# rrruko/squigly-trace

Hardware: AMD Instinct MI355X
Metric: Msamples/s (whole node) at 1080p/256spp on data/scene.obj (higher is better)
Workload: dtype f32; 1 GPU; data/scene.obj 1920x1080 @ 256 spp (BASELINE configs[1]), rows sharded over 1 GPU(s) in blocks of 2, RGB8 all_gather_into_tensor; row_block=2, nonblack_pixels=629970

## Files before the change

### squigly-trace_amd/csrc/sq_device.hip

```cpp
#include <hip/hip_runtime.h>

#include <algorithm>
#include <atomic>
#include <cmath>
#include <cstdlib>
#include <cstring>
#include <mutex>
#include <string>
#include <chrono>
#include <thread>
#include <vector>

#include "../../include/squigly_hip.h"
#include "../../include/squigly_host.h"
#include "sq_error.h"
#include "sq_pack.h"
#include "sq_kernels_lane.h"
#include "sq_kernels_wave.h"
#include "sq_kernels_trace.h"

#define SQ_HIP(expr)                                                                             \
    do {                                                                                         \
        hipError_t e_ = (expr);                                                                  \
        if (e_ != hipSuccess) return sq_set_error("%s failed: %s", #expr, hipGetErrorString(e_)); \
    } while (0)

constexpr int kOneshotRowBlock = 2;

struct RngTable { uint32_t* words = nullptr; size_t bytes = 0; int64_t cover = 0; hipEvent_t filled = nullptr; };
struct sq_device_scene {
    int device = 0;
    SceneView view{};
    void* d_arena = nullptr;
    int height = 0; bool small_index = false; int n_cu = 256;
    Level1Cull level1{};
    int shortcut_depth = 0;
    Work work{}; void* d_work = nullptr; size_t work_bytes = 0; int64_t work_pixels = 0, work_slots = 0;
    std::vector<std::pair<hipEvent_t, hipEvent_t>> pending;
    double total_ms = 0; int64_t launches = 0;
    Options opt;
    const char* last_kernel = "sq_trace_rays";
    sq_plan plan{}; bool has_plan = false;
    hipStream_t aux = nullptr; std::vector<hipEvent_t> events;
    float* d_cams = nullptr; int64_t cams_cap = 0;
    float* d_px_sum2 = nullptr; int64_t px_sum2_cap = 0;
    RngTable rng{};
    std::vector<sq_light> lights{ sq_light{ { 0.0f, 3.0f, -1.0f }, { 2.0f, 2.0f, 2.0f } } };
    bool lights_set = false, lights_staged = false;
    float* d_lights = nullptr; float* cast_carry = nullptr;
    int32_t depth = 3;
    void* d_deep = nullptr; size_t deep_bytes = 0;
    sq_sky sky{}; bool sky_set = false;
};

extern "C" int sq_scene_upload(const sq_scene* sc, int32_t device, sq_device_scene** out) {
    if (sq_check_scene_args(sc, out)) return 1;
    int ndev = 0;
    if (hipGetDeviceCount(&ndev) != hipSuccess || ndev < 1) return sq_set_error("no HIP device available (this library has no CPU fallback)");
    if (device < 0 || device >= ndev) return sq_set_error("device %d outside 0..%d", device, ndev - 1);
    PackedScene P;
    if (sq_pack_scene(*sc, P)) return 1;
    SQ_HIP(hipSetDevice(device));
    sq_device_scene* s = new sq_device_scene;
    s->device = device; s->height = P.height; s->small_index = P.small_index; s->shortcut_depth = P.shortcut_depth; s->level1 = P.level1;
    hipDeviceProp_t prop;
    if (hipGetDeviceProperties(&prop, device) == hipSuccess && prop.multiProcessorCount > 0) s->n_cu = prop.multiProcessorCount;
    SceneView& v = s->view;
    auto arrays = [&](auto&& f) {
        f(v.branches, P.branches, false); f(v.leaves, P.leaves, false); f(v.tris, P.tris, false); f(v.tri_mat, P.tri_mat, false);
        f(v.surfs, P.surfs, false); f(v.mats, P.mats, false); f(v.verts4, P.verts4, false); f(v.trix, P.trix, false);
        f(v.rbranch, P.rbranch, false); f(v.emitters, P.emitters, false);
        f(v.cull_child, P.cull_child, true); f(v.cull_child16, P.cull_child16, true); f(v.branches_m, P.branches_m, true);
    };
    auto slot = [](size_t bytes) { return ((bytes ? bytes : 16) + 255) & ~(size_t)255; };
    size_t arena_bytes = 0;
    arrays([&](auto&, const auto& vec, bool optional) { if (!optional || !vec.empty()) arena_bytes += slot(vec.size() * sizeof(vec[0])); });
    if (hipMalloc(&s->d_arena, arena_bytes) != hipSuccess) { sq_scene_free(s); return sq_set_error("hipMalloc(%zu) for the scene failed", arena_bytes); }
    std::vector<unsigned char> staging(arena_bytes, 0);
    size_t off = 0;
    arrays([&](auto& member, const auto& vec, bool optional) {
        if (optional && vec.empty()) return;
        const size_t bytes = vec.size() * sizeof(vec[0]);
        if (bytes) std::memcpy(staging.data() + off, vec.data(), bytes);
        member = reinterpret_cast<std::remove_reference_t<decltype(member)>>((const char*)s->d_arena + off);
        off += slot(bytes);
    });
    if (hipMemcpy(s->d_arena, staging.data(), arena_bytes, hipMemcpyHostToDevice) != hipSuccess) { sq_scene_free(s); return sq_set_error("hipMemcpy H2D of the scene failed"); }
    if (P.trix.empty()) v.trix = nullptr;
    for (int c = 0; c < 3; ++c) { v.root_lo[c] = sc->root.lo[c]; v.root_hi[c] = sc->root.hi[c]; }
    v.root_ref = P.root_ref; v.packed_leaves = P.packed_leaves; v.rroot = P.rroot;
    v.n_branches = P.nb; v.n_leaves = P.nl; v.n_tris = sc->n_tris; v.n_mats = sc->n_mats; v.n_verts = P.n_verts; v.n_emitters = P.n_emitters;
    v.height = P.height; v.nonneg_materials = P.nonneg_materials; v.finite_geometry = P.finite_geometry;
    v.cull_o2max = P.cull_limits[0]; v.cull_d2min = P.cull_limits[1]; v.cull_d2max = P.cull_limits[2];
    v.rtail = nullptr; v.incremental_ok = 0;
    *out = s;
    return 0;
}

namespace {
struct CachedBlock { void* ptr = nullptr; size_t bytes = 0; };
std::mutex g_cache_mutex;
CachedBlock g_cache[64];
void* cache_take(int device, size_t bytes, size_t* got) {
    std::lock_guard<std::mutex> lock(g_cache_mutex);
    CachedBlock& c = g_cache[device & 63];
    if (!c.ptr || c.bytes < bytes) return nullptr;
    void* p = c.ptr; *got = c.bytes; c = CachedBlock{};
    return p;
}
void cache_give(int device, void* ptr, size_t bytes) {
    void* drop = ptr;
    {
        std::lock_guard<std::mutex> lock(g_cache_mutex);
        CachedBlock& c = g_cache[device & 63];
        if (bytes > c.bytes) { drop = c.ptr; c.ptr = ptr; c.bytes = bytes; }
    }
    if (drop) (void)hipFree(drop);
}
RngTable g_rng_cache[64];
void rng_free(RngTable& t) {
    if (t.words) (void)hipFree(t.words);
    if (t.filled) (void)hipEventDestroy(t.filled);
    t = RngTable{};
}
bool rng_cache_take(int device, int64_t cover, RngTable* out) {
    std::lock_guard<std::mutex> lock(g_cache_mutex);
    RngTable& c = g_rng_cache[device & 63];
    if (!c.words || c.cover < cover) return false;
    *out = c; c = RngTable{};
    return true;
}
void rng_cache_give(int device, RngTable& t) {
    RngTable drop = t;
    t = RngTable{};
    {
        std::lock_guard<std::mutex> lock(g_cache_mutex);
        RngTable& c = g_rng_cache[device & 63];
        if (drop.cover > c.cover) std::swap(drop, c);
    }
    rng_free(drop);
}
}
extern "C" void sq_release_cached_memory(void) {
    for (int d = 0; d < 64; ++d) {
        size_t got = 0;
        void* p = cache_take(d, 0, &got);
        RngTable t;
// ... 1029 lines not shown
```

### squigly-trace_amd/csrc/sq_frame.h

```cpp
#pragma once
#include "sq_plan.h"
#include "sq_scene.h"

using sq::f3;
using namespace sqd;

struct Frame {
    float cam_pos[3]; float cam_rot[9];
    int32_t samples, w, h, cast;
    int32_t row_block, shard, n_shards, local_rows;
    int32_t tile_rows, tiles_x;
    float* out_avg; uint8_t* out_rgb;
    int32_t k_begin, k_end;
    float* sum;
    int32_t diag;
    int32_t n_views, view_pixels;
    const float* cams;
    const uint8_t* mask; float* sum2; int32_t* count;
};
struct RayFrame : Frame {
    const float* ray_org; const float* ray_dir; const long long* ray_seed;
};
template <int SRC> using FrameOf = std::conditional_t<SRC == kSrcRays, RayFrame, Frame>;
constexpr int kCamWords = 12;
// ... 85 lines not shown
template <typename T> __device__ __forceinline__ T sky_arg() { return T{}; }
template <typename T> __device__ __forceinline__ const T& sky_arg(const T& k) { return k; }
__device__ __forceinline__ float sky_t(f3 d) {
    const float n = sq::fsqrt((d.x * d.x + d.y * d.y) + d.z * d.z);
    const float u = d.z / n;
    return 0.5f * u + 0.5f;
}
__device__ __forceinline__ f3 sky_at(const Sky& K, float t) {
    return sq::mk(K.down[0] + t * (K.up[0] - K.down[0]), K.down[1] + t * (K.up[1] - K.down[1]), K.down[2] + t * (K.up[2] - K.down[2]));
}
__device__ __forceinline__ void store_fold(const Frame& F, long long pix, f3 sum) {
    if (F.sum) { float* o = F.sum + pix * 3; o[0] = sum.x; o[1] = sum.y; o[2] = sum.z; }
    const f3 avg = sq::scale(1 / (float)F.k_end, sum);
    if (F.out_avg) { float* o = F.out_avg + pix * 3; o[0] = avg.x; o[1] = avg.y; o[2] = avg.z; }
    if (F.out_rgb) tonemap(avg, F.out_rgb + pix * 3);
}
template <bool AD>
__device__ __forceinline__ void store_miss_sky(const Frame& F, long long pix, const Sky& K, f3 d0) {
    const f3 c = sky_at(K, sky_t(d0));
    f3 sum = fold_start(F, pix);
    for (int k = F.k_begin; k < F.k_end; ++k) sum = sum + c;
    if constexpr (AD) {
        if (F.sum2) {
            f3 sum2 = fold_start2(F, pix);
            for (int k = F.k_begin; k < F.k_end; ++k) sum2 = sum2 + c * c;
            float* o = F.sum2 + pix * 3; o[0] = sum2.x; o[1] = sum2.y; o[2] = sum2.z;
        }
        store_count(F, pix);
    }
    store_fold(F, pix, sum);
}

struct Work {
    int32_t* n_active;
    int32_t* px_pixel;
    float*   px_t0;
    int32_t* px_tri0;
    float*   px_sum;
    float*   px_mt;
    int32_t* px_mtri;
    uint8_t* state;
    float4*  org;
    float4*  dir;
    int32_t* tri1;
    int32_t* head[2];
    unsigned long long* stats;
    int64_t  slot_capacity;
    float*   px_sum2;
};
constexpr uint8_t kDone = 0, kRay1 = 1, kMirror = 2, kRay2 = 3;

constexpr int kDiagGauge = 24, kDiagWaves = 25, kDiagStartBeside = 26, kDiagEndBeside = 27;
constexpr int kStatLevel1Culled = 28;

__device__ __forceinline__ int wave_append(int32_t* counter, bool want) {
    const unsigned long long m = sq_ballot(want);
    if (m == 0) return -1;
    const int lane = threadIdx.x & 63;
    const int leader = __ffsll((long long)m) - 1;
    int base = 0;
    if (lane == leader) base = atomicAdd(counter, __popcll(m));
    base = __shfl(base, leader);
    return want ? base + __popcll(m & ((1ull << lane) - 1ull)) : -1;
}

template <bool AD>
__device__ __forceinline__ void store_active(const Frame& F, const Work& W, int a, long long pix, float t, int tri) {
    W.px_pixel[a] = (int32_t)pix; W.px_t0[a] = t; W.px_tri0[a] = tri;
    const f3 s0 = fold_start(F, pix);
    W.px_sum[3 * a] = s0.x; W.px_sum[3 * a + 1] = s0.y; W.px_sum[3 * a + 2] = s0.z;
    if constexpr (AD) {
        if (F.sum2) { const f3 q0 = fold_start2(F, pix); W.px_sum2[3 * a] = q0.x; W.px_sum2[3 * a + 1] = q0.y; W.px_sum2[3 * a + 2] = q0.z; }
        store_count(F, pix);
    }
}
template <bool AD>
__device__ __forceinline__ void store_miss(const Frame& F, long long pix) {
    if constexpr (AD) store_live_miss(F, pix); else store_miss_sum(F, pix);
}

constexpr int kRngRun = 4;
constexpr size_t kRngPad = 256;
struct RngView { const uint32_t* words; long long cover; };

__device__ __forceinline__ f3 level0_radiance(const Surface& s0) { return s0.surf * sq::mk(0, 0, 0) + s0.emit; }
struct Shade1 { f3 surf, emit; };
__device__ __forceinline__ Shade1 shade1_of(const SceneView& S, int tri) {
    const float4* q = S.surfs + 3 * (size_t)tri;
    return Shade1{ sq::mk(q[1].x, q[1].y, q[1].z), sq::mk(q[2].x, q[2].y, q[2].z) };
}
__device__ __forceinline__ f3 level1_radiance(const Surface& s0, const Shade1& s1) {
    const f3 L1 = s1.surf * sq::mk(0, 0, 0) + s1.emit;
    return s0.surf * L1 + s0.emit;
}

constexpr int kMaxDepth = kDeepestPath;
__device__ __forceinline__ uint32_t tf_word(const uint64_t c[4], int i) {
    const uint64_t w = i < 2 ? c[0] : i < 4 ? c[1] : i < 6 ? c[2] : c[3];
    return (i & 1) ? (uint32_t)(w >> 32) : (uint32_t)w;
}
__device__ __forceinline__ f3 path_radiance(const SceneView& S, const Surface& s0, const int (&tr)[kMaxDepth], f3 inner) {
    f3 L = inner;
#pragma unroll
    for (int b = kMaxDepth - 1; b >= 1; --b)
        if (tr[b] >= 0) { const Shade1 q = shade1_of(S, tr[b]); L = q.surf * L + q.emit; }
    return s0.surf * L + s0.emit;
// ... 40 lines not shown
```

### squigly-trace_amd/csrc/sq_host.cpp

```cpp
#include "../../include/squigly_host.h"
#include "sq_error.h"
#include "sq_host_types.h"
#include "sq_math.h"
#include "sq_pack.h"
#include "sq_plan.h"

#include <algorithm>
#include <cmath>
#include <cstdio>
#include <cstdlib>
#include <cstring>
#include <string>
#include <unordered_map>
#include <vector>

using sq::f3;

namespace {

struct Scanner {
    const char* s; size_t n; size_t i = 0;
    Scanner(const char* p, size_t len) : s(p), n(len) {}
    int peek() const { return i < n ? (unsigned char)s[i] : -1; }
    static bool ws(int c) { return c == ' ' || c == '\t' || c == '\n' || c == '\r' || c == '\f' || c == '\v'; }
// ... 713 lines not shown
                vmax2 = std::max(vmax2, q);
            }
        const double vmax = std::sqrt(vmax2), omax = 2.0 * vmax * (1.0 + 1e-12);
        double g1 = 0.0;
        for (int32_t i = 0; i < sc.n_tris; ++i) {
            if (emits[(size_t)i]) continue;
            const TriNorms q = tri_norms(sc.tris[i]);
            if (!(q.P <= kLemmaPmax)) return;
            const double rho = lemma_rho(q, omax), r = 7.0 * u * q.P / eps;
            g1 = std::max(g1, rho + 1.01 * (r * (omax + vmax + rho) + rho));
        }
        const double delta1 = 4.0 * u * (2.0 * (vmax + g1) + omax) * (1.0 + 1e-6), R1 = vmax + g1 + delta1;
        if (!(R1 <= 1048576.0)) return;
        double six = 0.0;
        for (int c = 0; c < 3; ++c) { L.em_lo[c] = P.emitters.empty() ? 0.0 : 1e300; L.em_hi[c] = P.emitters.empty() ? 0.0 : -1e300; }
        for (int32_t e : P.emitters) {
            const sq_tri& t = sc.tris[e];
            const TriNorms q = tri_norms(t);
            if (!(q.P <= kLemmaPmax)) return;
            L.em_rho = std::max(L.em_rho, 32.0 * (u / eps) * q.P * (R1 + q.V0 + q.E1 + q.E2));
            six = std::max(six, 6.0 * u * (q.E1 + q.E2));
            for (const float* v : { t.v0, t.v1, t.v2 })
                for (int c = 0; c < 3; ++c) {
                    L.em_lo[c] = std::min(L.em_lo[c], (double)v[c]);
                    L.em_hi[c] = std::max(L.em_hi[c], (double)v[c]);
                }
        }
        L.em_add = six + delta1 + 1e-20;
        std::vector<float> vals;
        for (int32_t i = 0; i < sc.n_tris; ++i) vals.push_back(P.surfs[(size_t)i].reflective);
        std::sort(vals.begin(), vals.end()); vals.erase(std::unique(vals.begin(), vals.end()), vals.end());
        const size_t nv = vals.size(), nc = std::min<size_t>(nv, (size_t)kLevel1Classes);
        L.n_classes = (int32_t)nc;
        for (size_t c = 0; c < nc; ++c) {
            L.class_val[c] = vals[nv - nc + c];
            const float from = (c == 0) ? vals[0] : L.class_val[c];
            float* b = L.class_box[c];
            b[0] = b[1] = b[2] = INFINITY; b[3] = b[4] = b[5] = -INFINITY;
            for (int32_t i = 0; i < sc.n_tris; ++i) {
                if (!(P.surfs[(size_t)i].reflective >= from)) continue;
                const sq_tri& t = sc.tris[i];
                const TriNorms q = tri_norms(t);
                if (!(q.P <= kLemmaPmax)) { b[0] = b[1] = b[2] = -INFINITY; b[3] = b[4] = b[5] = INFINITY; break; }
                double m = lemma_rho(q, omax);
                m += 8.0 * u * (vmax_inf + m + omax) + 1e-20;
                for (int k = 0; k < 3; ++k) {
                    const double lo = std::min({ (double)t.v0[k], (double)t.v1[k], (double)t.v2[k] }), hi = std::max({ (double)t.v0[k], (double)t.v1[k], (double)t.v2[k] });
                    b[k] = std::min(b[k], f_down(lo - m)); b[3 + k] = std::max(b[3 + k], f_up(hi + m));
                }
            }
        }
        L.o2max = P.cull_limits[0]; L.d2min = P.cull_limits[1]; L.d2max = P.cull_limits[2];
        L.on = 1;
    }
    void geometry_flags() {
        bool fin = finite3(sc.root.lo) && finite3(sc.root.hi);
        for (const DevBranch& d : P.branches) fin = fin && finite3(d.lo) && finite3(d.hi) && finite(d.lmax) && finite(d.rmin);
        for (int32_t i = 0; i < sc.n_tris && fin; ++i) fin = finite3(sc.tris[i].v0) && finite3(sc.tris[i].v1) && finite3(sc.tris[i].v2);
        P.finite_geometry = fin;
        P.small_index = P.nb < 0x8000 && sc.n_tris < 0x8000;
        P.n_verts = (int32_t)(P.verts4.size() / 4);
    }
};

}

int sq_pack_scene(const sq_scene& sc, PackedScene& out) {
    out = PackedScene{};
    Packer k{ sc, out };
    if (validate_tree(sc, out.height, k.depth)) return 1;
    if (sc.height && sc.height != out.height) return sq_set_error("scene.height = %d but the tree has height %d", sc.height, out.height);
    k.renumber(); k.branch_boxes(); k.material_flags(); k.triangles_and_surfaces(); k.vertex_index_form(); k.resident_encoding();
    if (k.culling_tables() || k.leaf_references()) return 1;
    k.merged_records(); k.emitter_list(); k.geometry_flags(); k.level1_tables();
    return 0;
}

struct sq_packed : PackedScene {};
extern "C" int sq_scene_pack(const sq_scene* sc, sq_packed** out) {
    if (sq_check_scene_args(sc, out)) return 1;
    sq_packed* p = new sq_packed;
    if (sq_pack_scene(*sc, *p)) { delete p; return 1; }
    *out = p;
    return 0;
}
extern "C" void sq_packed_free(sq_packed* p) { delete p; }
extern "C" int sq_packed_array(const sq_packed* P, const char* name, const void** data, size_t* bytes) {
    if (!P || !name || !data || !bytes) return sq_set_error("null argument");
    bool found = false;
    auto is = [&](const char* n, const auto& v) { if (!found && !std::strcmp(name, n)) { found = true; *data = v.data(); *bytes = v.size() * sizeof(v[0]); } };
    is("branches", P->branches); is("leaves", P->leaves); is("tris", P->tris); is("tri_mat", P->tri_mat); is("surfs", P->surfs);
    is("mats", P->mats); is("verts4", P->verts4); is("trix", P->trix); is("rbranch", P->rbranch); is("emitters", P->emitters);
    is("cull_child", P->cull_child); is("cull_child16", P->cull_child16); is("branches_m", P->branches_m);
    if (!found && !std::strcmp(name, "level1")) { found = true; *data = &P->level1; *bytes = sizeof P->level1; }
    return found ? 0 : sq_set_error("no packed array '%s'", name);
}
extern "C" int sq_packed_scalar(const sq_packed* P, const char* name, int64_t* value) {
    if (!P || !name || !value) return sq_set_error("null argument");
    uint32_t lim[3]; std::memcpy(lim, P->cull_limits, sizeof lim);
    const struct { const char* name; int64_t value; } all[] = {
        { "n_branches", P->nb }, { "n_leaves", P->nl }, { "height", P->height }, { "root_ref", P->root_ref }, { "rroot", P->rroot },
        { "packed_leaves", P->packed_leaves }, { "nonneg_materials", P->nonneg_materials }, { "finite_geometry", P->finite_geometry },
        { "n_emitters", P->n_emitters }, { "n_verts", P->n_verts }, { "cull_o2max", lim[0] }, { "cull_d2min", lim[1] }, { "cull_d2max", lim[2] },
        { "small_index", P->small_index }, { "shortcut_depth", P->shortcut_depth }, { "level1_zero", P->level1_zero }, { "level1_on", P->level1.on } };
    for (const auto& s : all) if (!std::strcmp(name, s.name)) { *value = s.value; return 0; }
    return sq_set_error("no packed scalar '%s'", name);
}

extern "C" int64_t sq_rng_table_cover(int32_t w, int32_t h, int32_t samples, int64_t budget_bytes) {
    if (w < 1 || h < 1 || samples < 1 || budget_bytes < 12) return 0;
    const unsigned __int128 span = (unsigned __int128)samples * ((unsigned __int128)(w - 1) * (unsigned __int128)w + (unsigned __int128)h);
    const unsigned __int128 cap = (unsigned __int128)(budget_bytes / 12);
    return (int64_t)(span < cap ? span : cap);
}

namespace sqd {
namespace {
enum OptionKind { kAny, kRange, kBool, kSign, kIgnored };
struct OptionRow { const char* name; int64_t Options::* member; OptionKind kind; int64_t lo, hi; const char* refusal; };
const OptionRow kOptionTable[] = {
    { "timing", &Options::timing, kAny, 0, 0, nullptr },
    { "variant", &Options::variant, kRange, 1, 2, "variant must be 1 (per-pixel kernel) or 2 (wavefront)" },
    { "slots", &Options::slots, kRange, 1, 512ll << 20, "slots must be in 1..2^29" },
    { "straggler_lanes", &Options::straggler_lanes, kRange, 0, 63, "straggler_lanes must be in 0..63" },
    { "resident", &Options::resident, kBool, 0, 1, nullptr },
    { "profile", &Options::profile, kBool, 0, 1, nullptr },
    { "lds_node_kb", &Options::lds_node_kb, kRange, 0, 128, "lds_node_kb must be in 0..128" },
    { "trace_blocks_per_cu", &Options::trace_blocks_per_cu, kRange, 0, 8, "trace_blocks_per_cu must be in 0..8" },
    { "overlap", &Options::overlap, kRange, 0, 2, "overlap must be 0, 1 or 2" },
    { "rng_table_mb", &Options::rng_table_mb, kRange, 0, 1ll << 20, "rng_table_mb must be in 0..2^20" },
    { "cast_wavefront", &Options::cast_wavefront, kBool, 0, 1, nullptr },
    { "deep", &Options::deep, kBool, 0, 1, nullptr },
    { "pool", &Options::pool, kBool, 0, 1, nullptr },
    { "guided", &Options::guided, kRange, 0, 3, "guided must be in 0..3" },
    { "primary_resident", &Options::primary_resident, kBool, 0, 1, nullptr },
    { "cull", &Options::cull, kBool, 0, 1, nullptr },
    { "level1_cull", &Options::level1_cull, kBool, 0, 1, nullptr },
    { "incremental", nullptr, kIgnored, 0, 0, nullptr },
    { "primary_tiles", &Options::primary_tiles, kBool, 0, 1, nullptr },
    { "primary_pooled", &Options::primary_pooled, kBool, 0, 1, nullptr },
    { "coresidency", &Options::coresidency, kBool, 0, 1, nullptr },
    { "aux_polite", &Options::aux_polite, kRange, 0, 8, "aux_polite must be in 0..8" },
    { "trace_prio", &Options::trace_prio, kRange, 0, 3, "trace_prio must be in 0..3" },
    { "aux_low_priority", &Options::aux_low_priority, kBool, 0, 1, nullptr },
    { "descend_extra", &Options::descend_extra, kRange, 0, 16, "descend_extra must be in 0..16" },
    { "descend_lanes", &Options::descend_lanes, kRange, 1, 64, "descend_lanes must be in 1..64" },
// ... 306 lines not shown
```

### squigly-trace_amd/csrc/sq_kernels_wave.h

```cpp
#pragma once
#include "sq_frame.h"

__device__ __forceinline__ void diag_aux_wave(const Work& W, int diag, bool at_start) {
    if (!diag || (threadIdx.x & 63) != 0) return;
    const unsigned long long live = atomicAdd(&W.stats[kDiagGauge], 0ull);
    if (at_start) atomicAdd(&W.stats[kDiagWaves], 1ull);
    if (live >= (unsigned long long)diag) atomicAdd(&W.stats[at_start ? kDiagStartBeside : kDiagEndBeside], 1ull);
}

template <typename StackT, int SRC, bool AD, bool SKY, typename FrameT>
__device__ __forceinline__ void primary_body(const SceneView& S, const FrameT& F, const Work& W, const Sky& K) {
    constexpr bool MV = SRC == kSrcViews;
    extern __shared__ float4 lds_raw[];
    SQ_LDS StackT* stk = to_lds<StackT>(lds_raw) + threadIdx.x;
    const long long q = (long long)blockIdx.x * kBlock + threadIdx.x;
    int view = 0;
    long long pix;
    if constexpr (SRC == kSrcRays) pix = q < (long long)F.h ? q : -1;
    else if constexpr (MV) pix = q < primary_padded(F) * F.n_views ? primary_tile_views(F, q, view) : -1;
    else pix = q < primary_padded(F) ? primary_tile(F, q) : -1;
    bool in = pix >= 0;
    if constexpr (AD) in = in && pixel_live(F, pix);
    Hit h0; h0.tri = -1; h0.t = 0;
    f3 d0 = sq::mk(0, 0, 0);
// ... 50 lines not shown
__device__ __forceinline__ long long seed_base(const FrameT& F, const Work& W, int a, const Pixel0& P) {
    if constexpr (SRC == kSrcRays) return F.ray_seed[W.px_pixel[a]];
    else return (long long)F.samples * ((long long)P.x + (long long)P.y * (long long)F.w);
}
__device__ __forceinline__ bool absorbs(const SceneView& S, const Surface& s) {
    return S.nonneg_materials && s.surf.x == 0.0f && s.surf.y == 0.0f && s.surf.z == 0.0f;
}
__device__ __forceinline__ void finish_level1(const Work& W, long long sid, int tri1) {
    W.tri1[sid] = tri1;
    W.state[sid] = kDone;
}
__device__ __forceinline__ int2 slot_hit(const float4& org) { return make_int2(__float_as_int(org.x), __float_as_int(org.y)); }

struct RngRun { uint32_t w[3 * kRngRun]; };
__device__ __forceinline__ RngRun rng_load_run(const uint32_t* words, long long seed) {
    RngRun r;
    const uint32_t* p = words + 3 * seed;
    if ((seed & 3) == 0) {
        const uint4* q = reinterpret_cast<const uint4*>(p);
        const uint4 a = q[0], b = q[1], c = q[2];
        r.w[0] = a.x; r.w[1] = a.y; r.w[2] = a.z; r.w[3] = a.w; r.w[4] = b.x; r.w[5] = b.y; r.w[6] = b.z; r.w[7] = b.w;
        r.w[8] = c.x; r.w[9] = c.y; r.w[10] = c.z; r.w[11] = c.w;
    } else {
#pragma unroll
        for (int i = 0; i < 3 * kRngRun; ++i) r.w[i] = p[i];
    }
    return r;
}
__global__ void __launch_bounds__(kBlock) sq_rng_fill(uint32_t* words, long long quad_begin, long long quad_end) {
    for (long long q = quad_begin + (long long)blockIdx.x * kBlock + threadIdx.x; q < quad_end; q += (long long)gridDim.x * kBlock) {
        uint32_t w[3 * kRngRun];
#pragma unroll
        for (int j = 0; j < kRngRun; ++j) sq::tfgen3(q * kRngRun + j, w[3 * j], w[3 * j + 1], w[3 * j + 2]);
        uint4* o = reinterpret_cast<uint4*>(words + 3 * kRngRun * q);
        o[0] = make_uint4(w[0], w[1], w[2], w[3]); o[1] = make_uint4(w[4], w[5], w[6], w[7]); o[2] = make_uint4(w[8], w[9], w[10], w[11]);
    }
}

__device__ __forceinline__ bool halfplane_misses_box(f3 p0, f3 d1, f3 nd, const double* lo, const double* hi, double m) {
    const double px[3] = { p0.x, p0.y, p0.z }, dx[3] = { d1.x, d1.y, d1.z }, nx[3] = { nd.x, nd.y, nd.z };
    double g[3], h[3], scale = 0.0;
#pragma unroll
    for (int k = 0; k < 3; ++k) { g[k] = 0.5 * (lo[k] + hi[k]) - px[k]; h[k] = 0.5 * (hi[k] - lo[k]) + m; scale += __builtin_fabs(g[k]) + h[k]; }
    const double tol = 1e-9 * scale;
    const double N[3] = { dx[1] * nx[2] - dx[2] * nx[1], dx[2] * nx[0] - dx[0] * nx[2], dx[0] * nx[1] - dx[1] * nx[0] };
    const double dist = __builtin_fabs(N[0] * g[0] + N[1] * g[1] + N[2] * g[2]);
    const double rad = __builtin_fabs(N[0]) * h[0] + __builtin_fabs(N[1]) * h[1] + __builtin_fabs(N[2]) * h[2];
    if (dist > rad + tol) return true;
    const double f = (dx[0] * nx[0] + dx[1] * nx[1] + dx[2] * nx[2]) / (nx[0] * nx[0] + nx[1] * nx[1] + nx[2] * nx[2]);
    const double w[3] = { dx[0] - f * nx[0], dx[1] - f * nx[1], dx[2] - f * nx[2] };
    const double side = w[0] * g[0] + w[1] * g[1] + w[2] * g[2] + __builtin_fabs(w[0]) * h[0] + __builtin_fabs(w[1]) * h[1] + __builtin_fabs(w[2]) * h[2];
    return side < -tol;
}
__device__ __forceinline__ bool level1_culled(const SceneView& S, const Level1Cull& C, bool p0_ok, f3 p0, f3 d1, uint32_t n1, uint32_t n2) {
    const float eps = 0.0001f, inf = __builtin_inff();
    const f3 df = sq::mk(1.0f / d1.x, 1.0f / d1.y, 1.0f / d1.z);
    const f3 nodf = sq::mk(-p0.x * df.x, -p0.y * df.y, -p0.z * df.z);
    const float dd = sq::dot(d1, d1);
    if (!(p0_ok && finite3(d1) && finite3(df) && finite3(nodf) && dd >= C.d2min && dd <= C.d2max)) return false;
    const float un1 = sq::unit_float(n1);
    bool has = false; float b[6] = { 0, 0, 0, 0, 0, 0 };
#pragma unroll
    for (int c = kLevel1Classes - 1; c >= 0; --c) {
        if (c < C.n_classes && C.class_val[c] >= un1) {
            has = true;
#pragma unroll
            for (int k = 0; k < 6; ++k) b[k] = C.class_box[c][k];
        }
    }
    if (has && cull_slab(b, df, nodf)) return false;
    const f3 nd = random_vector(n1, n2);
    const float nn = sq::dot(nd, nd);
    if (!(nn >= C.d2min && nn <= C.d2max)) return false;
    float amin = inf;
    for (int j = 0; j < S.n_emitters; ++j) {
        const float* tp = S.tris + 9 * (size_t)S.emitters[j];
        const f3 v0 = sq::mk(tp[0], tp[1], tp[2]), e1 = sq::mk(tp[3], tp[4], tp[5]), e2 = sq::mk(tp[6], tp[7], tp[8]);
        float t_unused;
        if (moller_trumbore(p0, d1, v0, e1, e2, t_unused)) return false;
        const float a = sq::dot(e1, sq::cross(nd, e2));
        if (!(a > -eps && a < eps)) amin = sq::hmin(amin, __builtin_fabsf(a));
    }
    if (amin == inf) return true;
    if (!(amin < inf)) return false;
    return halfplane_misses_box(p0, d1, nd, C.em_lo, C.em_hi, C.em_rho * ((double)eps / (double)amin) + C.em_add);
}

template <int SRC, typename FrameT>
__device__ __forceinline__ void gen_bounce1_body(const SceneView& S, const FrameT& F, const Work& W, int k_base, int k_count, const RngView R, const Level1Cull& C) {
    const int A = *W.n_active;
    unsigned int n_culled = 0;
    diag_aux_wave(W, F.diag, true);
    const int n_runs = (k_count + kRngRun - 1) / kRngRun, runs_per_y = (n_runs + (int)gridDim.y - 1) / (int)gridDim.y;
    const int g_begin = min(n_runs, (int)blockIdx.y * runs_per_y), g_end = min(n_runs, g_begin + runs_per_y);
    for (int a = blockIdx.x * kBlock + threadIdx.x; a < A; a += gridDim.x * kBlock) {
        const Pixel0 P = load_pixel0<SRC>(S, F, W, a);
        const long long rix = seed_base<SRC>(F, W, a, P);
        if (absorbs(S, P.s0)) {
            for (int kl = g_begin * kRngRun; kl < min(k_count, g_end * kRngRun); ++kl) W.state[(long long)kl * A + a] = kDone;
            continue;
        }
        const long long first = rix + k_base;
        const bool use = R.words != nullptr && rix >= 0 && rix <= R.cover - (long long)F.samples;
        const bool p0_ok = C.on && finite3(P.p0) && sq::dot(P.p0, P.p0) <= C.o2max;
        RngRun next{};
        if (use && g_begin < g_end) next = rng_load_run(R.words, first + (long long)g_begin * kRngRun);
        for (int g = g_begin; g < g_end; ++g) {
            RngRun cur = next;
            if (use && g + 1 < g_end) next = rng_load_run(R.words, first + (long long)(g + 1) * kRngRun);
#pragma unroll 1
            for (int kl = g * kRngRun; kl < min(k_count, (g + 1) * kRngRun); ++kl) {
                const long long sid = (long long)kl * A + a;
                uint32_t n0, n1, n2;
                if (use) {
                    n0 = cur.w[0]; n1 = cur.w[1]; n2 = cur.w[2];
#pragma unroll
                    for (int i = 0; i + 3 < 3 * kRngRun; ++i) cur.w[i] = cur.w[i + 3];
                } else {
                    long long seed = first + kl;
                    asm volatile("" : "+v"(seed));
                    sq::tfgen3(seed, n0, n1, n2);
                }
                if (!scatters(P.s0, n0)) {
                    W.state[sid] = kMirror;
                    *reinterpret_cast<float2*>(reinterpret_cast<float*>(W.org + sid) + 2) = make_float2(__uint_as_float(n2), __uint_as_float(n1));
                    continue;
                }
                const f3 d1 = scatter_dir(P.d0, P.s0, n0, n1);
                if (C.on && level1_culled(S, C, p0_ok, P.p0, d1, n1, n2)) { finish_level1(W, sid, -1); ++n_culled; continue; }
                W.state[sid] = kRay1;
                W.org[sid] = make_float4(P.p0.x, P.p0.y, P.p0.z, __uint_as_float(n1));
                W.dir[sid] = make_float4(d1.x, d1.y, d1.z, __uint_as_float(n2));
            }
        }
    }
    if (C.on) {
#pragma unroll
        for (int o = 32; o > 0; o >>= 1) n_culled += __shfl_xor(n_culled, o);
        if ((threadIdx.x & 63) == 0 && n_culled) atomicAdd(&W.stats[kStatLevel1Culled], (unsigned long long)n_culled);
    }
    diag_aux_wave(W, F.diag, false);
}
constexpr int kGen1Waves = 4;
template <int SRC>
__global__ void __launch_bounds__(kBlock, kGen1Waves) sq_gen_bounce1(const SceneView S, const FrameOf<SRC> F, const Work W, int k_base, int k_count, const RngView R, const Level1Cull C) { gen_bounce1_body<SRC>(S, F, W, k_base, k_count, R, C); }

template <int SRC, typename FrameT>
__device__ __forceinline__ void mirror1_gen_body(const SceneView& S, const FrameT& F, const Work& W, long long base) {
    const int A = *W.n_active;
    for (int a = blockIdx.x * kBlock + threadIdx.x; a < A; a += gridDim.x * kBlock) {
        const Pixel0 P = load_pixel0<SRC>(S, F, W, a);
        const long long sl = base + a;
        if (absorbs(S, P.s0)) { W.state[sl] = kDone; continue; }
        const f3 d1 = mirror_dir(P.d0, P.s0);
        W.state[sl] = kRay1;
        W.org[sl] = make_float4(P.p0.x, P.p0.y, P.p0.z, 0.0f);
        W.dir[sl] = make_float4(d1.x, d1.y, d1.z, 0.0f);
    }
}
template <int SRC>
__global__ void __launch_bounds__(kBlock) sq_mirror1_gen(const SceneView S, const FrameOf<SRC> F, const Work W, long long base) { mirror1_gen_body<SRC>(S, F, W, base); }
__global__ void __launch_bounds__(kBlock) sq_mirror1_store(const Work W, long long base) {
    const int A = *W.n_active;
    for (int a = blockIdx.x * kBlock + threadIdx.x; a < A; a += gridDim.x * kBlock) {
        const bool live = W.state[base + a] == kRay1;
        const int2 hit = slot_hit(W.org[base + a]);
        W.px_mt[a] = live ? __int_as_float(hit.x) : 0.0f;
        W.px_mtri[a] = live ? hit.y : -1;
    }
}

template <int SRC, bool AD>
__global__ void __launch_bounds__(kBlock) sq_primary_gen(const FrameOf<SRC> F, const Work W, long long total) {
    if (blockIdx.x == 0 && threadIdx.x == 0) W.n_active[48] = (int32_t)total;
    for (long long pix = (long long)blockIdx.x * kBlock + threadIdx.x; pix < total; pix += (long long)gridDim.x * kBlock) {
        if constexpr (AD) { if (!pixel_live(F, pix)) { W.state[pix] = kDone; continue; } }
        if constexpr (SRC == kSrcRays) {
            const f3 o = load3(F.ray_org, pix), d = load3(F.ray_dir, pix);
            W.state[pix] = kRay1;
            W.org[pix] = make_float4(o.x, o.y, o.z, 0.0f);
            W.dir[pix] = make_float4(d.x, d.y, d.z, 0.0f);
        } else if constexpr (SRC == kSrcViews) {
            int y, x;
            const ViewCam c = view_cam<false>(F, view_coords(F, (int)pix, y, x));
            const f3 d = primary_dir(c.rot, F.w, F.h, y, x);
            W.state[pix] = kRay1;
            W.org[pix] = make_float4(c.pos.x, c.pos.y, c.pos.z, 0.0f);
            W.dir[pix] = make_float4(d.x, d.y, d.z, 0.0f);
        } else {
            int y, x;
            pixel_coords(F, pix, y, x);
            const f3 d = primary_dir(F.cam_rot, F.w, F.h, y, x);
// ... 413 lines not shown
```

### squigly-trace_amd/csrc/sq_layout.h

```cpp
#pragma once
#include <stdint.h>
namespace sqd {
constexpr uint32_t kLeafBit = 0x80000000u;

struct DevBranch {
    float lo[3]; float lmax;
    float hi[3]; float rmin;
    float lmax2, rmin2;
    uint32_t left, right;
};
struct DevLeaf { int32_t first, count; };
struct DevTri {
    float v0[3];
    float e1[3];
    float e2[3];
};
struct DevMat { float reflective, sr, sg, sb, emissive, er, eg, eb; };
struct DevSurf {
    float n[3], reflective;
    float surf[3], pad0;
    float emit[3], pad1;
};
static_assert(sizeof(DevBranch) == 48 && sizeof(DevLeaf) == 8 && sizeof(DevTri) == 36 && sizeof(DevMat) == 32 && sizeof(DevSurf) == 48,
              "the device records have the sizes their comments promise");

constexpr int kAxisShift = 29;
constexpr uint32_t kAxisMask = 3u << kAxisShift;
constexpr uint32_t kGrownLeft = 1u, kGrownRight = 2u;
constexpr int kLevel1Classes = 4;
struct Level1Cull {
    int32_t on;
    int32_t n_classes;
    float o2max, d2min, d2max;
    float class_val[kLevel1Classes];
    float class_box[kLevel1Classes][6];
    double em_lo[3], em_hi[3];
    double em_rho, em_add;
};
constexpr int kTriRunPad = 3;
}
```

### squigly-trace_amd/csrc/sq_pack.h

```cpp
#pragma once
#include <cstdint>
#include <vector>

#include "../../include/squigly_hip.h"
#include "sq_layout.h"

constexpr int kDeepestPath = 8;

struct PackedScene {
    std::vector<sqd::DevBranch> branches;
    std::vector<sqd::DevLeaf> leaves;
    std::vector<sqd::DevTri> tris;
    std::vector<int32_t> tri_mat;
    std::vector<sqd::DevSurf> surfs;
    std::vector<sqd::DevMat> mats;
    std::vector<float> verts4;
    std::vector<uint16_t> trix;
    std::vector<uint32_t> rbranch;
    std::vector<int32_t> emitters;
    std::vector<float> cull_child;
    std::vector<uint32_t> cull_child16;
    std::vector<uint32_t> branches_m;
    int32_t nb = 0, nl = 0, height = 0;
    uint32_t root_ref = 0, rroot = 0;
    bool packed_leaves = false, nonneg_materials = false, finite_geometry = false;
    int32_t n_emitters = -1, n_verts = 0;
    int32_t shortcut_depth = 0;
    float cull_limits[3] = { -1.0f, 0.25f, 1.5624f };
    sqd::Level1Cull level1{};
    bool level1_zero = false;
    bool small_index = false;
};

int sq_check_scene_args(const sq_scene* sc, const void* out);
int sq_pack_scene(const sq_scene& sc, PackedScene& out);
```

Measured before the change: 12790 Msamples/s.

## Cull first-bounce rays whose path stretch misses a conservative box cover of occluders

Adds a host-built cover of up to eight conservative boxes around all non-emissive triangles, inflated by error bounds, and uploads it as a scene array. On the device, the level-1 cull now also finds the parameter interval where the ray can still reach the emitter half-plane region. If that interval intersects none of the cover boxes, the bounce is terminated early and counted in a new stat. The aim is to skip more second-ray traversals at the cost of extra double and float box tests per scattered ray and a pairwise greedy box merge at load time.

Measured after the change: 13400 Msamples/s (median of 6 runs). 4.7% higher.

```diff
diff --git a/squigly-trace_amd/csrc/sq_device.hip b/squigly-trace_amd/csrc/sq_device.hip
--- a/squigly-trace_amd/csrc/sq_device.hip
+++ b/squigly-trace_amd/csrc/sq_device.hip
@@ -71,6 +71,7 @@
         f(v.surfs, P.surfs, false); f(v.mats, P.mats, false); f(v.verts4, P.verts4, false); f(v.trix, P.trix, false);
         f(v.rbranch, P.rbranch, false); f(v.emitters, P.emitters, false);
         f(v.cull_child, P.cull_child, true); f(v.cull_child16, P.cull_child16, true); f(v.branches_m, P.branches_m, true);
+        f(v.rtail, P.level1_cover, true);
     };
     auto slot = [](size_t bytes) { return ((bytes ? bytes : 16) + 255) & ~(size_t)255; };
     size_t arena_bytes = 0;
@@ -92,7 +93,7 @@
     v.n_branches = P.nb; v.n_leaves = P.nl; v.n_tris = sc->n_tris; v.n_mats = sc->n_mats; v.n_verts = P.n_verts; v.n_emitters = P.n_emitters;
     v.height = P.height; v.nonneg_materials = P.nonneg_materials; v.finite_geometry = P.finite_geometry;
     v.cull_o2max = P.cull_limits[0]; v.cull_d2min = P.cull_limits[1]; v.cull_d2max = P.cull_limits[2];
-    v.rtail = nullptr; v.incremental_ok = 0;
+    v.incremental_ok = 0;
     *out = s;
     return 0;
 }
diff --git a/squigly-trace_amd/csrc/sq_frame.h b/squigly-trace_amd/csrc/sq_frame.h
--- a/squigly-trace_amd/csrc/sq_frame.h
+++ b/squigly-trace_amd/csrc/sq_frame.h
@@ -161,6 +161,7 @@
 
 constexpr int kDiagGauge = 24, kDiagWaves = 25, kDiagStartBeside = 26, kDiagEndBeside = 27;
 constexpr int kStatLevel1Culled = 28;
+constexpr int kStatLevel1Stretch = 29;
 
 __device__ __forceinline__ int wave_append(int32_t* counter, bool want) {
     const unsigned long long m = sq_ballot(want);
diff --git a/squigly-trace_amd/csrc/sq_host.cpp b/squigly-trace_amd/csrc/sq_host.cpp
--- a/squigly-trace_amd/csrc/sq_host.cpp
+++ b/squigly-trace_amd/csrc/sq_host.cpp
@@ -789,6 +789,80 @@
         }
         L.o2max = P.cull_limits[0]; L.d2min = P.cull_limits[1]; L.d2max = P.cull_limits[2];
         L.on = 1;
+        level1_cover(emits, omax, 8.0 * u * (vmax_inf * (1.0 + 1e-6) + g1 + omax) + 1e-20);
+    }
+    void level1_cover(const std::vector<char>& emits, double omax, double slab_slack) {
+        const double u = kLemmaU, eps = kLemmaEps;
+        struct Box { double lo[3], hi[3], r, c; int64_t count; int axis; int64_t cell; };
+        auto join = [](const Box& a, const Box& b) {
+            Box o = a; o.count += b.count; o.r = std::max(a.r, b.r); o.c = std::max(a.c, b.c);
+            for (int k = 0; k < 3; ++k) { o.lo[k] = std::min(a.lo[k], b.lo[k]); o.hi[k] = std::max(a.hi[k], b.hi[k]); }
+            return o;
+        };
+        auto volume = [](const Box& a) { return (a.hi[0] - a.lo[0]) * (a.hi[1] - a.lo[1]) * (a.hi[2] - a.lo[2]); };
+        std::vector<Box> each;
+        double slo[3] = { 1e300, 1e300, 1e300 }, shi[3] = { -1e300, -1e300, -1e300 };
+        for (int32_t i = 0; i < sc.n_tris; ++i) {
+            if (emits[(size_t)i]) continue;
+            const sq_tri& t = sc.tris[i];
+            const TriNorms q = tri_norms(t);
+            const double rho = lemma_rho(q, omax);
+            double e1[3], e2[3];
+            for (int k = 0; k < 3; ++k) { e1[k] = (double)(t.v1[k] - t.v0[k]); e2[k] = (double)(t.v2[k] - t.v0[k]); }
+            const double n[3] = { e1[1] * e2[2] - e1[2] * e2[1], e1[2] * e2[0] - e1[0] * e2[2], e1[0] * e2[1] - e1[1] * e2[0] };
+            const double nn = std::sqrt(n[0] * n[0] + n[1] * n[1] + n[2] * n[2]);
+            Box b{}; b.count = 1; b.axis = 3; b.cell = 0;
+            b.r = 7.0 * u * q.P / eps; b.c = 8.0 * u * (omax + q.V0) * q.E1 * q.E2 / eps;
+            for (int k = 0; k < 3; ++k) {
+                const double across = std::sqrt(n[(k + 1) % 3] * n[(k + 1) % 3] + n[(k + 2) % 3] * n[(k + 2) % 3]);
+                const double s = nn > 1e-6 * q.E1 * q.E2 ? std::min(1.0, across / nn + 1e-6) : 1.0;
+                const double pts[5] = { (double)t.v0[k], (double)t.v1[k], (double)t.v2[k], (double)t.v0[k] + e1[k], (double)t.v0[k] + e2[k] };
+                b.lo[k] = *std::min_element(pts, pts + 5) - rho * s - slab_slack;
+                b.hi[k] = *std::max_element(pts, pts + 5) + rho * s + slab_slack;
+                slo[k] = std::min(slo[k], b.lo[k]); shi[k] = std::max(shi[k], b.hi[k]);
+            }
+            each.push_back(b);
+        }
+        const double extent = each.empty() ? 0.0 : std::max({ shi[0] - slo[0], shi[1] - slo[1], shi[2] - slo[2] });
+        for (Box& b : each) {
+            const double ex[3] = { b.hi[0] - b.lo[0], b.hi[1] - b.lo[1], b.hi[2] - b.lo[2] }, longest = std::max({ ex[0], ex[1], ex[2] });
+            for (int k = 2; k >= 0; --k) if (ex[k] <= 1e-4 * extent && ex[k] < 0.05 * longest) b.axis = k;
+            if (b.axis < 3) b.cell = (int64_t)std::floor(0.5 * (b.lo[b.axis] + b.hi[b.axis]) / std::max(1e-3 * extent, 1e-300) + 0.5);
+            else for (int k = 0; k < 3; ++k) b.cell |= (int64_t)(b.lo[k] + b.hi[k] >= slo[k] + shi[k]) << k;
+        }
+        std::stable_sort(each.begin(), each.end(), [](const Box& a, const Box& b) { return a.axis != b.axis ? a.axis < b.axis : a.cell < b.cell; });
+        std::vector<Box> boxes, octants;
+        for (size_t i = 0; i < each.size(); ++i) {
+            std::vector<Box>& to = each[i].axis < 3 ? boxes : octants;
+            if (i && each[i].axis == each[i - 1].axis && each[i].cell == each[i - 1].cell) to.back() = join(to.back(), each[i]);
+            else to.push_back(each[i]);
+        }
+        constexpr size_t kMaxGroups = 56;
+        if (boxes.size() > kMaxGroups) {
+            std::stable_sort(boxes.begin(), boxes.end(), [](const Box& a, const Box& b) { return a.count > b.count; });
+            for (size_t i = kMaxGroups; i < boxes.size(); ++i) octants.push_back(boxes[i]);
+            boxes.resize(kMaxGroups);
+        }
+        boxes.insert(boxes.end(), octants.begin(), octants.end());
+        while (boxes.size() > (size_t)kLevel1Boxes) {
+            size_t bi = 0, bj = 1; double best = INFINITY;
+            for (size_t i = 0; i < boxes.size(); ++i)
+                for (size_t j = i + 1; j < boxes.size(); ++j) {
+                    const double grow = volume(join(boxes[i], boxes[j])) - volume(boxes[i]) - volume(boxes[j]);
+                    if (grow < best) { best = grow; bi = i; bj = j; }
+                }
+            boxes[bi] = join(boxes[bi], boxes[bj]);
+            boxes.erase(boxes.begin() + (std::ptrdiff_t)bj);
+        }
+        if (boxes.empty()) return;
+        Level1Cover V{};
+        V.n = (int32_t)boxes.size();
+        for (size_t j = 0; j < (size_t)kLevel1Boxes; ++j) {
+            const Box& b = boxes[j < boxes.size() ? j : 0];
+            V.r[j] = f_up(b.r + 2e-6); V.c[j] = f_up(b.c * (1.0 + 1e-5) + 1e-30);
+            for (int k = 0; k < 3; ++k) { V.box[j][k] = f_down(b.lo[k]); V.box[j][3 + k] = f_up(b.hi[k]); }
+        }
+        P.level1_cover.assign(1, V);
     }
     void geometry_flags() {
         bool fin = finite3(sc.root.lo) && finite3(sc.root.hi);
@@ -828,7 +902,7 @@
     auto is = [&](const char* n, const auto& v) { if (!found && !std::strcmp(name, n)) { found = true; *data = v.data(); *bytes = v.size() * sizeof(v[0]); } };
     is("branches", P->branches); is("leaves", P->leaves); is("tris", P->tris); is("tri_mat", P->tri_mat); is("surfs", P->surfs);
     is("mats", P->mats); is("verts4", P->verts4); is("trix", P->trix); is("rbranch", P->rbranch); is("emitters", P->emitters);
-    is("cull_child", P->cull_child); is("cull_child16", P->cull_child16); is("branches_m", P->branches_m);
+    is("cull_child", P->cull_child); is("cull_child16", P->cull_child16); is("branches_m", P->branches_m); is("level1_cover", P->level1_cover);
     if (!found && !std::strcmp(name, "level1")) { found = true; *data = &P->level1; *bytes = sizeof P->level1; }
     return found ? 0 : sq_set_error("no packed array '%s'", name);
 }
diff --git a/squigly-trace_amd/csrc/sq_kernels_wave.h b/squigly-trace_amd/csrc/sq_kernels_wave.h
--- a/squigly-trace_amd/csrc/sq_kernels_wave.h
+++ b/squigly-trace_amd/csrc/sq_kernels_wave.h
@@ -126,7 +126,57 @@
     const double side = w[0] * g[0] + w[1] * g[1] + w[2] * g[2] + __builtin_fabs(w[0]) * h[0] + __builtin_fabs(w[1]) * h[1] + __builtin_fabs(w[2]) * h[2];
     return side < -tol;
 }
-__device__ __forceinline__ bool level1_culled(const SceneView& S, const Level1Cull& C, bool p0_ok, f3 p0, f3 d1, uint32_t n1, uint32_t n2) {
+#ifndef SQ_LEVEL1_COVER
+#define SQ_LEVEL1_COVER 1
+#endif
+__device__ __forceinline__ bool stretch_misses_cover(f3 p0, f3 d1, f3 nd, const double* lo, const double* hi, double m, const uint4* cover) {
+    const double px[3] = { p0.x, p0.y, p0.z }, dx[3] = { d1.x, d1.y, d1.z }, nx[3] = { nd.x, nd.y, nd.z };
+    double g[3], h[3], scale = 0.0;
+#pragma unroll
+    for (int k = 0; k < 3; ++k) { g[k] = 0.5 * (lo[k] + hi[k]) - px[k]; h[k] = 0.5 * (hi[k] - lo[k]) + m; scale += __builtin_fabs(g[k]) + h[k]; }
+    const double tol = 1e-9 * scale;
+    const double N[3] = { dx[1] * nx[2] - dx[2] * nx[1], dx[2] * nx[0] - dx[0] * nx[2], dx[0] * nx[1] - dx[1] * nx[0] };
+    const double G[3] = { g[1] * nx[2] - g[2] * nx[1], g[2] * nx[0] - g[0] * nx[2], g[0] * nx[1] - g[1] * nx[0] };
+    const double r[3] = { __builtin_fabs(nx[2]) * h[1] + __builtin_fabs(nx[1]) * h[2], __builtin_fabs(nx[2]) * h[0] + __builtin_fabs(nx[0]) * h[2],
+                          __builtin_fabs(nx[1]) * h[0] + __builtin_fabs(nx[0]) * h[1] };
+    bool use[3]; double Nu[3];
+#pragma unroll
+    for (int k = 0; k < 3; ++k) { use[k] = __builtin_fabs(N[k]) >= 1e-6; Nu[k] = use[k] ? N[k] : 1.0; }
+    const double inv = 1.0 / ((Nu[0] * Nu[1]) * Nu[2]);
+    const double rc[3] = { inv * (Nu[1] * Nu[2]), inv * (Nu[0] * Nu[2]), inv * (Nu[0] * Nu[1]) };
+    double ta = 0.0, tb = (double)__builtin_inff();
+#pragma unroll
+    for (int k = 0; k < 3; ++k) {
+        const double w = r[k] + tol;
+        const double q1 = (G[k] - w) * rc[k], q2 = (G[k] + w) * rc[k];
+        const double ql = __builtin_fmin(q1, q2), qh = __builtin_fmax(q1, q2);
+        ta = use[k] ? __builtin_fmax(ta, ql - 1e-9 * __builtin_fabs(ql)) : ta;
+        tb = use[k] ? __builtin_fmin(tb, qh + 1e-9 * __builtin_fabs(qh)) : tb;
+    }
+    if (ta > tb) return true;
+    if (!SQ_LEVEL1_COVER || cover == nullptr) return false;
+    const float ta32 = ta > 1e-30 ? (float)(ta * (1.0 - 0x1p-20)) : 0.0f, tb32 = (float)(tb * (1.0 + 0x1p-20));
+    f3 dh = d1;
+    asm volatile("" : "+v"(dh.x), "+v"(dh.y), "+v"(dh.z));
+    const f3 df = sq::mk(1.0f / dh.x, 1.0f / dh.y, 1.0f / dh.z);
+    const f3 nodf = sq::mk(-p0.x * df.x, -p0.y * df.y, -p0.z * df.z);
+    const __attribute__((address_space(4))) float* V = (const __attribute__((address_space(4))) float*)cover;
+    bool may_end = false;
+#pragma unroll
+    for (int j = 0; j < kLevel1Boxes; ++j) {
+        const float rj = V[4 + j], cj = V[4 + kLevel1Boxes + j];
+        const __attribute__((address_space(4))) float* b = V + 4 + 2 * kLevel1Boxes + 6 * j;
+        const float t1 = __builtin_fmaf(b[0], df.x, nodf.x), t2 = __builtin_fmaf(b[3], df.x, nodf.x);
+        const float t3 = __builtin_fmaf(b[1], df.y, nodf.y), t4 = __builtin_fmaf(b[4], df.y, nodf.y);
+        const float t5 = __builtin_fmaf(b[2], df.z, nodf.z), t6 = __builtin_fmaf(b[5], df.z, nodf.z);
+        const float tmin = vmax3(vmin(t1, t2), vmin(t3, t4), vmin(t5, t6));
+        const float tmax = vmin3(vmax(t1, t2), vmax(t3, t4), vmax(t5, t6));
+        const float tlo = (tmin - rj * __builtin_fabsf(tmin)) - cj, thi = (tmax + rj * __builtin_fabsf(tmax)) + cj;
+        may_end |= vmax(tlo, ta32) <= vmin(thi, tb32);
+    }
+    return !may_end;
+}
+__device__ __forceinline__ int level1_culled(const SceneView& S, const Level1Cull& C, bool p0_ok, f3 p0, f3 d1, uint32_t n1, uint32_t n2) {
     const float eps = 0.0001f, inf = __builtin_inff();
     const f3 df = sq::mk(1.0f / d1.x, 1.0f / d1.y, 1.0f / d1.z);
     const f3 nodf = sq::mk(-p0.x * df.x, -p0.y * df.y, -p0.z * df.z);
@@ -155,15 +205,17 @@
         const float a = sq::dot(e1, sq::cross(nd, e2));
         if (!(a > -eps && a < eps)) amin = sq::hmin(amin, __builtin_fabsf(a));
     }
-    if (amin == inf) return true;
-    if (!(amin < inf)) return false;
-    return halfplane_misses_box(p0, d1, nd, C.em_lo, C.em_hi, C.em_rho * ((double)eps / (double)amin) + C.em_add);
+    if (amin == inf) return 1;
+    if (!(amin < inf)) return 0;
+    const double m = C.em_rho * ((double)eps / (double)amin) + C.em_add;
+    if (halfplane_misses_box(p0, d1, nd, C.em_lo, C.em_hi, m)) return 1;
+    return stretch_misses_cover(p0, d1, nd, C.em_lo, C.em_hi, m, S.rtail) ? 2 : 0;
 }
 
 template <int SRC, typename FrameT>
 __device__ __forceinline__ void gen_bounce1_body(const SceneView& S, const FrameT& F, const Work& W, int k_base, int k_count, const RngView R, const Level1Cull& C) {
     const int A = *W.n_active;
-    unsigned int n_culled = 0;
+    unsigned int n_culled = 0, n_culled4 = 0;
     diag_aux_wave(W, F.diag, true);
     const int n_runs = (k_count + kRngRun - 1) / kRngRun, runs_per_y = (n_runs + (int)gridDim.y - 1) / (int)gridDim.y;
     const int g_begin = min(n_runs, (int)blockIdx.y * runs_per_y), g_end = min(n_runs, g_begin + runs_per_y);
@@ -201,7 +253,10 @@
                     continue;
                 }
                 const f3 d1 = scatter_dir(P.d0, P.s0, n0, n1);
-                if (C.on && level1_culled(S, C, p0_ok, P.p0, d1, n1, n2)) { finish_level1(W, sid, -1); ++n_culled; continue; }
+                if (C.on) {
+                    const int why = level1_culled(S, C, p0_ok, P.p0, d1, n1, n2);
+                    if (why) { finish_level1(W, sid, -1); n_culled += why == 1; n_culled4 += why == 2; continue; }
+                }
                 W.state[sid] = kRay1;
                 W.org[sid] = make_float4(P.p0.x, P.p0.y, P.p0.z, __uint_as_float(n1));
                 W.dir[sid] = make_float4(d1.x, d1.y, d1.z, __uint_as_float(n2));
@@ -210,8 +265,9 @@
     }
     if (C.on) {
 #pragma unroll
-        for (int o = 32; o > 0; o >>= 1) n_culled += __shfl_xor(n_culled, o);
+        for (int o = 32; o > 0; o >>= 1) { n_culled += __shfl_xor(n_culled, o); n_culled4 += __shfl_xor(n_culled4, o); }
         if ((threadIdx.x & 63) == 0 && n_culled) atomicAdd(&W.stats[kStatLevel1Culled], (unsigned long long)n_culled);
+        if ((threadIdx.x & 63) == 0 && n_culled4) atomicAdd(&W.stats[kStatLevel1Stretch], (unsigned long long)n_culled4);
     }
     diag_aux_wave(W, F.diag, false);
 }
diff --git a/squigly-trace_amd/csrc/sq_layout.h b/squigly-trace_amd/csrc/sq_layout.h
--- a/squigly-trace_amd/csrc/sq_layout.h
+++ b/squigly-trace_amd/csrc/sq_layout.h
@@ -37,5 +37,12 @@
     double em_lo[3], em_hi[3];
     double em_rho, em_add;
 };
+constexpr int kLevel1Boxes = 8;
+struct Level1Cover {
+    int32_t n; int32_t pad[3];
+    float r[kLevel1Boxes], c[kLevel1Boxes];
+    float box[kLevel1Boxes][6];
+};
+static_assert(sizeof(Level1Cover) == 272, "the cover is seventeen 16-byte quads");
 constexpr int kTriRunPad = 3;
 }
diff --git a/squigly-trace_amd/csrc/sq_pack.h b/squigly-trace_amd/csrc/sq_pack.h
--- a/squigly-trace_amd/csrc/sq_pack.h
+++ b/squigly-trace_amd/csrc/sq_pack.h
@@ -28,6 +28,7 @@
     int32_t shortcut_depth = 0;
     float cull_limits[3] = { -1.0f, 0.25f, 1.5624f };
     sqd::Level1Cull level1{};
+    std::vector<sqd::Level1Cover> level1_cover;
     bool level1_zero = false;
     bool small_index = false;
 };
```
